# kaylode/vehicle-counting

Hardware: AMD Instinct MI355X
Metric: end-to-end frames/sec (detect+NMS+ReID+track), YOLOv5s 640px (higher is better)
Workload: dtype bf16; 1 GPU; YOLOv5s 640x640 single camera stream per GPU, bf16 convs (BASELINE.json configs[1]); workload_id=s640-bf16, clip_frames=512, objects=12, num_classes=80, detection_injection=False, weights=seeded synthetic (no checkpoints available), streams=1, ranks=1, counts_allgather_via=vc_allgather_counts (RCCL, C ABI), tracked_rows=155352, tracker=device-resident (one kernel per batch, no host round trip per frame)

## Files before the change

include/vcount_hip.h:

```cpp
#ifndef VCOUNT_HIP_H
#define VCOUNT_HIP_H

#include <stddef.h>
#include <stdint.h>

#ifdef __cplusplus
extern "C" {
#endif

#define VC_OK 0
#define VC_ERR_ARG 1
#define VC_ERR_HIP 2
#define VC_ERR_STATE 3
#define VC_ERR_CAPACITY 4
#define VC_ERR_NOTFOUND 5

#define VC_PREC_BF16 0
#define VC_PREC_F32 1
#define VC_PREC_FP8 2

#define VC_FEAT_DIM 512
#define VC_REID_SIZE 50

int vc_version(void);
// ... 88 lines not shown
    int full_range;
    int pitch_y, pitch_c;
    size_t offset_c, offset_v, frame_stride;
} vc_yuv_desc;
int vc_yuv_desc_default(vc_yuv_desc* d);
int vc_stream_stage_yuv_host(vc_engine* e, const vc_yuv_desc* d, const uint8_t* yuv_host, int b, int h, int w, void** frames_dev_out);
int vc_stream_stage_yuv_dev(vc_engine* e, const vc_yuv_desc* d, const void* yuv_dev, int b, int h, int w, void** frames_dev_out);
int vc_yuv_to_bgr_dev(const vc_yuv_desc* d, const void* yuv_dev, int b, int h, int w, void* bgr_dev);

int vc_stream_run_async(vc_engine* e, const int* trackers, int num_classes, const void* frames_dev, int b, int h, int w,
                        int cap_rows_per_frame);
int vc_stream_collect(vc_engine* e, int64_t* out_rows6, int cap_rows_per_frame, int* out_m, int* out_ndet, int b);
int vc_stream_run_async_multi(vc_engine* e, const int* trackers , int n_cam, int num_classes, const int* cam_of_frame ,
                              const void* frames_dev, int b, int h, int w, int cap_rows_per_frame);
int vc_stream_reset(vc_engine* e);

int vc_stream_embed(vc_engine* e, const void* frames_dev, int b, int h, int w, double* out_rows7, int cap_rows, int* out_n, const float** out_feat_dev);
int vc_allgather_rows(vc_engine* e, const double* rows7, const float* feat_dev, int n, double* out_rows7, int cap_rows, int* out_counts ,
                      const float** out_feat_dev);
int vc_videotracker_run_features(vc_engine* e, const int* trackers, int num_classes, const double* rows7, const float* feat_dev, int n, int h, int w,
                                 int64_t* out_rows6, int cap_rows_per_frame, int* out_m, int64_t* out_keys, int cap_frames, int* out_n_frames);
int vc_stream_inject(vc_engine* e, const float* det6 , const int* count, int b, int n);

typedef struct vc_counter vc_counter;
int vc_counter_create(const double* polygon_xy, int n_points, const double* dir_lines, int n_dir, int num_classes, vc_counter** out);
int vc_counter_destroy(vc_counter* c);
int vc_counter_add(vc_counter* c, const int64_t* frames, const int64_t* track_ids, const int64_t* labels, const int64_t* boxes_xyxy, int n);
int vc_counter_tracks(const vc_counter* c, int* n);
int vc_counts(const vc_counter* c, int32_t* out );
int vc_counter_rows_count(const vc_counter* c, int64_t* n);
// ... 74 lines not shown
```

vehicle-counting_amd/_lib.py:

```python
from __future__ import annotations

import ctypes as C
import os

import numpy as np

_HERE = os.path.dirname(os.path.abspath(__file__))
os.environ.setdefault("GPU_MAX_HW_QUEUES", "8")
LIB_PATH = os.environ.get("VC_LIB_PATH") or os.path.join(_HERE, "libvcount_hip.so")

VC_OK = 0
PREC_BF16, PREC_F32, PREC_FP8 = 0, 1, 2
PREC_ID = {"bf16": 0, "f32": 1, "fp8": 2}
NET_YOLO, NET_REID = 0, 1
FEAT_DIM = 512
PROF_CONV, PROF_DETECT_AUX, PROF_REID_AUX, PROF_TRACK = 0, 1, 2, 3
PIX_ID = {"nv12": 0, "i420": 1}
YUV_MATRIX_ID = {"bt601": 0, "bt709": 1}
RENDER_SRC_ID = {"bgr_host": 0, "bgr_dev": 1, "yuv_host": 2, "yuv_dev": 3}


class VcError(RuntimeError):
    def __init__(self, code, msg):
        super().__init__(f"libvcount_hip status {code}: {msg}")
# ... 72 lines not shown
    "vc_yuv_desc_default": [_P(YuvDesc)],
    "vc_stream_stage_yuv_host": [_vp, _P(YuvDesc), _vp, _i, _i, _i, _P(_vp)],
    "vc_stream_stage_yuv_dev": [_vp, _P(YuvDesc), _vp, _i, _i, _i, _P(_vp)],
    "vc_yuv_to_bgr_host": [_P(YuvDesc), _pu8, _i, _i, _i, _pu8],
    "vc_yuv_to_bgr_dev": [_P(YuvDesc), _vp, _i, _i, _i, _vp],
    "vc_bgr_to_yuv_host": [_P(YuvDesc), _pu8, _i, _i, _i, _pu8],
    "vc_bgr_to_yuv_dev": [_P(YuvDesc), _vp, _i, _i, _i, _vp],
    "vc_render_create": [_vp, _i, _i, _i, _i, _P(_vp)],
    "vc_render_destroy": [_vp],
    "vc_render_submit": [_vp, _P(RenderSrc), _i, _i, _i, _pi, _pi, _P(YuvDesc), _vp, _i],
    "vc_render_collect": [_vp],
    "vc_stream_run_async": [_vp, _pi, _i, _vp, _i, _i, _i, _i],
    "vc_stream_collect": [_vp, _pl, _i, _pi, _pi, _i],
    "vc_stream_run_async_multi": [_vp, _pi, _i, _i, _pi, _vp, _i, _i, _i, _i],
    "vc_stream_reset": [_vp],
    "vc_stream_embed": [_vp, _vp, _i, _i, _i, _pd, _i, _pi, _P(_vp)],
    "vc_allgather_rows": [_vp, _pd, _vp, _i, _pd, _i, _pi, _P(_vp)],
    "vc_videotracker_run_features": [_vp, _pi, _i, _pd, _vp, _i, _i, _i, _pl, _i, _pi, _pl, _i, _pi],
    "vc_counter_create": [_pd, _i, _pd, _i, _i, _P(_vp)],
    "vc_counter_destroy": [_vp],
    "vc_counter_add": [_vp, _pl, _pl, _pl, _pl, _i],
    "vc_counter_tracks": [_vp, _pi],
    "vc_counts": [_vp, _pi],
    "vc_counter_rows_count": [_vp, _pl],
    "vc_counter_rows": [_vp, C.c_int64, _pl, _pl, _pl, _pl, _pi, _pd, _pd, _pl, _pl],
    "vc_comm_unique_id": [_vp],
    "vc_comm_init": [_vp, _i, _i, _vp],
    "vc_comm_destroy": [_vp],
    "vc_allgather_counts": [_vp, _pi, _i, _pi],
    "vc_overlay": [_vp, _vp, _i, _i, _i, _pi, _pi],
# ... 68 lines not shown
```

vehicle-counting_amd/csrc/engine.h:

```cpp
#pragma once
#include <chrono>
#include <condition_variable>
#include <deque>
#include <map>
#include <mutex>
#include <memory>
#include <string>
#include <vector>

#include "kernels.h"

namespace vc {

struct ConvParam {
    std::string name;
    int O = 0, I = 0, kh = 0, kw = 0;
    bool set = false;
    bool pair_stem = false;
    int fuse_a = -1, fuse_b = -1;
    int obj_of = -1;
    bool hidden = false;
    std::vector<float> w, b;
    void* d_w = nullptr;
    float* d_scale = nullptr;
// ... 64 lines not shown
    std::vector<TrackTaskHost> tasks;
    std::vector<int> dev_index;
    std::vector<std::pair<int, int>> tracker_dets;
    std::vector<int> last_task_of;
};

struct YuvGeom {
    int nv12, h, w, pitch_y, pitch_c;
    size_t off_c, off_v, frame_stride, frame_end;
    int yoff, cy, cvr, cvg, cug, cub;
    int matrix, full_range;
};

}

struct vc_render;

struct vc_engine {
    vc_engine_config cfg{};
    int prec = 0;
    int aux_prec = 0;
    float act_scale = 1.0f;
    hipStream_t stream = nullptr;
    hipStream_t dstream = nullptr;
    hipStream_t rstream = nullptr;
    hipStream_t hstream = nullptr;
    hipEvent_t ev_fork = nullptr, ev_join = nullptr;
    void* d_zero = nullptr; size_t zero_bytes = 0; bool want_hc_count = false;
    hipEvent_t ev_det[2] = {nullptr, nullptr};
    hipEvent_t ev_reid[3] = {nullptr, nullptr, nullptr};
    bool finalized = false;
    struct Options { int c3_fused = 1, bneck_fused = 1, bneck_cv3 = 1, front_fused = 1, crop_per_pixel = 0, sparse_head = 1, ff_ablate = 0, c3_ablate = 0, reid_block_fused = 1, head_side = 1, fuse_upsample = 1, sppf_sep = 1, fuse_s2_pw = 1; } opt;
    std::vector<void*> allocs;
    std::vector<void*> host_allocs;

    vc::Net yolo;
    int ch[5] = {0, 0, 0, 0, 0}, rep[4] = {0, 0, 0, 0};
    std::map<std::string, vc::View> ybuf;
    const vc::YoloPlan* last_plan = nullptr;
    std::vector<vc::ConvP> s2pw_folded;
    std::vector<std::pair<vc::View, vc::View>> up_folded;
    std::map<std::vector<int>, vc::YoloPlan> yolo_plans;
    std::map<std::pair<int, int>, vc::ReidPlan> reid_plans;
    uint8_t* d_frames = nullptr;
    size_t d_frames_bytes = 0;
    float* d_logits[3] = {nullptr, nullptr, nullptr};
    void* d_obj[3] = {nullptr, nullptr, nullptr};
// ... 22 lines not shown
    float* h_geom = nullptr;
    unsigned geom_seq = 0, submit_seq = 0;
    hipStream_t cstream = nullptr;
    uint8_t* d_ingest[4] = {nullptr, nullptr, nullptr, nullptr};
    hipEvent_t ev_ingest[4] = {nullptr, nullptr, nullptr, nullptr};
    unsigned ingest_seq = 0;
    bool ingest_staged[4] = {false, false, false, false};
    uint8_t* d_yuv_raw[4] = {nullptr, nullptr, nullptr, nullptr};
    size_t yuv_raw_bytes[4] = {0, 0, 0, 0};
    float* d_feat2[3] = {nullptr, nullptr, nullptr};
    int* d_crops2[3] = {nullptr, nullptr, nullptr};
    int* h_crops2[3] = {nullptr, nullptr, nullptr};
    unsigned reid_seq = 0;
    std::vector<int> crop_scratch;
    struct FrameDets { std::vector<double> xyxy, conf; std::vector<int> label; };
    struct Pending {
        const void* frames; int b, h, w, slot;
        int stage = 0;
        bool embed_refused = false;
        int fslot = 0;
        std::vector<FrameDets> fd;
        std::vector<int> row0;
        std::vector<float> inj_det; std::vector<int> inj_cnt; int inj_b = 0, inj_n = 0;
    };
    std::vector<Pending> pending;
    struct AsyncJob { int stage = 0, b = 0, cap = 0; std::vector<int> ndet; const void* frames = nullptr; };
    std::deque<AsyncJob> jobs;

    vc::Net reid;
    std::map<std::string, vc::View> rbuf;
    int* d_crops = nullptr;
    int* h_crops = nullptr;
    float* d_feat = nullptr;
    float* h_feat = nullptr;
    float* d_reid_in_nchw = nullptr;

    vc::TrackPool pool{};
// ... 76 lines not shown
int ingest_publish(vc_engine* e, int slot, void** frames_dev_out);
int yuv_resolve(const vc_yuv_desc* d, int b, int h, int w, YuvGeom& g);
size_t yuv_batch_bytes(const YuvGeom& g, int b);
int launch_yuv_to_bgr(const YuvGeom& g, const uint8_t* src, uint8_t* dst, int b, hipStream_t s);
int launch_bgr_to_yuv(const YuvGeom& g, const uint8_t* src_bgr, uint8_t* dst_yuv, int b, hipStream_t s);
int overlay_check_lists(int b, const int32_t* prims12, const int32_t* frame_first);
int launch_overlay(uint8_t* frames_dev, int b, int h, int w, const void* d_prims, const int* d_first, hipStream_t s);
void render_destroy_all(vc_engine* e);
struct ProfScope {
    vc_engine* e; int cat; double flops, bytes;
    hipStream_t s;
    ProfScope(vc_engine* e_, int cat_, double flops_ = 0, double bytes_ = 0, hipStream_t s_ = nullptr);
    ~ProfScope();
};
int tracker_init_pool(vc_engine* e);
struct Prepared { std::vector<double> tlwh, conf; std::vector<int> feat_rows; };
void prepare_dets(const double* xyxy, const double* conf, const int* rows, int k, const vc_tracker_params& p, Prepared& out);
void dsort_nms(const double* tlwh, const double* scores, int n, double max_overlap, std::vector<int>& keep);
struct FrameClassDets { int label, tracker; Prepared dets; };
int track_enqueue(vc_engine* e, int st, const std::vector<std::vector<FrameClassDets>>& frames, const float* d_feat, int W, int H,
                  int rows_cap, hipEvent_t wait);
int track_collect(vc_engine* e, int st, int64_t* out_rows6, int cap_rows_per_frame, int* out_m);
int track_idle(vc_engine* e);
int async_wait_all(vc_engine* e);
int frame_track(vc_engine* e, const uint8_t* d_frame_base, int frame_index, int H, int W, const std::vector<int>& tracker_ids,
                const std::vector<int>& labels, const std::vector<std::vector<int>>& groups, const double* xyxy, const double* conf,
                int n, std::vector<int64_t>& rows6);
}
```

vehicle-counting_amd/csrc/engine.hip:

```cpp
#include <algorithm>
#include <cmath>
#include <cstdarg>
#include <cstdlib>

#include "engine.h"

namespace vc {

static thread_local char g_err[1024] = "";
void set_error(const char* fmt, ...) {
    va_list ap;
    va_start(ap, fmt);
    vsnprintf(g_err, sizeof(g_err), fmt, ap);
    va_end(ap);
}
const char* last_error() { return g_err; }

int dev_alloc(vc_engine* e, void** p, size_t bytes) {
    if (bytes == 0) bytes = 16;
    VC_HIP(hipMalloc(p, bytes));
    e->allocs.push_back(*p);
    return VC_OK;
}
int dev_realloc(vc_engine* e, void** p, size_t bytes) {
// ... 128 lines not shown
    }
    int ndev = 0;
    VC_HIP(hipGetDeviceCount(&ndev));
    VC_CHECK(cfg->device >= 0 && cfg->device < ndev, VC_ERR_HIP, "device %d not present (%d visible)", cfg->device, ndev);
    VC_HIP(hipSetDevice(cfg->device));
    vc_engine* e = new vc_engine();
    e->cfg = *cfg;
    e->prec = cfg->precision;
    e->aux_prec = cfg->precision == VC_PREC_FP8 ? (int)PREC_BF16 : cfg->precision;
    e->act_scale = getenv("VC_FP8_ACT_SCALE") ? (float)atof(getenv("VC_FP8_ACT_SCALE")) : 1.0f;
    {
        auto env_int = [](const char* name, int dflt) { const char* v = getenv(name); return v ? atoi(v) : dflt; };
        e->opt.c3_fused = env_int("VC_C3_FUSED", 1); e->opt.bneck_fused = env_int("VC_BNECK_FUSED", 1); e->opt.bneck_cv3 = env_int("VC_BNECK_CV3", 1);
        e->opt.front_fused = env_int("VC_FRONT_FUSED", 1); e->opt.crop_per_pixel = getenv("VC_CROP_PER_PIXEL") ? 1 : 0;
        e->opt.sparse_head = env_int("VC_SPARSE_HEAD", 1); e->opt.reid_block_fused = env_int("VC_REID_BLOCK_FUSED", 1); e->opt.head_side = env_int("VC_HEAD_SIDE", 1); e->opt.fuse_upsample = env_int("VC_FUSE_UPSAMPLE", 1); e->opt.sppf_sep = env_int("VC_SPPF_SEP", 1); e->opt.fuse_s2_pw = env_int("VC_FUSE_S2PW", 1);
    }
    memcpy(e->anchors, kAnchors, sizeof(kAnchors));
    int st = VC_OK;
    do {
        int plo = 0, phi = 0;
        hipDeviceGetStreamPriorityRange(&plo, &phi);
        const int reserve = getenv("VC_TRACK_CUS") ? atoi(getenv("VC_TRACK_CUS")) : 0;
        bool ok;
        if (reserve > 0) {
            hipDeviceProp_t prop;
            hipGetDeviceProperties(&prop, cfg->device);
            const int ncu = prop.multiProcessorCount, words = (ncu + 31) / 32;
            std::vector<uint32_t> mt(words, 0), mc(words, 0);
            for (int c = 0; c < ncu; ++c) (c < reserve ? mt : mc)[c / 32] |= 1u << (c % 32);
            ok = hipExtStreamCreateWithCUMask(&e->stream, words, mt.data()) == hipSuccess &&
// ... 139 lines not shown
    }
    for (auto& p : e->reid.params) VC_TRY(pack_and_upload(e, p, e->aux_prec));
    e->d_frames_bytes = (size_t)e->cfg.max_batch * e->cfg.max_frame_h * e->cfg.max_frame_w * 3;
    VC_TRY(dev_alloc(e, (void**)&e->d_frames, e->d_frames_bytes));
    if (e->cfg.with_detector) VC_TRY(yolo_alloc(e));
    if (e->cfg.with_reid) VC_TRY(reid_alloc(e));
    for (auto& p : e->yolo.params) { p.w.clear(); p.w.shrink_to_fit(); }
    for (auto& p : e->reid.params) { p.w.clear(); p.w.shrink_to_fit(); }
    e->finalized = true;
    return VC_OK;
}

int vc_engine_set_option(vc_engine* e, const char* name, int value) {
    VC_CHECK(e && name, VC_ERR_ARG, "null argument");
    const std::string n = name;
    if (n == "c3_fused") e->opt.c3_fused = value;
    else if (n == "bneck_fused") e->opt.bneck_fused = value;
    else if (n == "bneck_cv3") e->opt.bneck_cv3 = value;
    else if (n == "front_fused") e->opt.front_fused = value;
    else if (n == "crop_per_pixel") e->opt.crop_per_pixel = value;
    else if (n == "sparse_head") e->opt.sparse_head = value;
    else if (n == "reid_block_fused") e->opt.reid_block_fused = value;
    else if (n == "head_side") e->opt.head_side = value;
    else if (n == "fuse_upsample") e->opt.fuse_upsample = value;
    else if (n == "sppf_sep") e->opt.sppf_sep = value;
    else if (n == "fuse_s2_pw") e->opt.fuse_s2_pw = value;
    else if (n == "ff_ablate") e->opt.ff_ablate = value;
    else if (n == "c3_ablate") e->opt.c3_ablate = value;
    else if (n == "dot_arena_mb") { VC_CHECK(value >= 0, VC_ERR_ARG, "dot_arena_mb must be >= 0"); e->dot_arena_max_floats = (size_t)value * 262144; }
    else { set_error("unknown option '%s'", name); return VC_ERR_NOTFOUND; }
// ... 407 lines not shown
```

vehicle-counting_amd/csrc/stream.hip:

```cpp
#include <algorithm>
#include <cmath>
#include <numeric>

#include <chrono>
#include <cstdlib>
#include <thread>

#include "engine.h"

using namespace vc;

namespace {
struct Tm {
    double acc[8] = {0, 0, 0, 0, 0, 0, 0, 0};
    long calls = 0;
    std::chrono::steady_clock::time_point t;
    bool on = getenv("VC_TIMING") != nullptr;
    void start() { if (on) t = std::chrono::steady_clock::now(); }
    void lap(int i) {
        if (!on) return;
        auto n = std::chrono::steady_clock::now();
        acc[i] += std::chrono::duration<double, std::micro>(n - t).count();
        t = n;
    }
// ... 103 lines not shown
    VC_TRY(ingest_take_slot(e, b, h, w, &slot));
    VC_HIP(hipMemcpyAsync(e->d_ingest[slot], frames_host, (size_t)b * h * w * 3, hipMemcpyHostToDevice, e->cstream));
    return ingest_publish(e, slot, frames_dev_out);
}

int vc_stream_submit_host(vc_engine* e, const uint8_t* frames_host, int b, int h, int w, void** frames_dev_out) {
    VC_CHECK(e && e->pending.size() < 2, e ? VC_ERR_STATE : VC_ERR_ARG, "two submissions are already in flight: call vc_stream_run first");
    VC_TRY(vc_stream_stage_host(e, frames_host, b, h, w, frames_dev_out));
    return vc_stream_submit(e, *frames_dev_out, b, h, w);
}

}

namespace {

int issue_reid(vc_engine* e, vc_engine::Pending& pd) {
    const int md = e->cfg.max_det, b = pd.b, h = pd.h, w = pd.w;
    const float* h_det = e->h_det2[pd.slot];
    const int* h_cnt = e->h_det_count2[pd.slot];
    pd.fd.assign(b, FrameDets{});
    pd.row0.assign(b, 0);
    for (int f = 0; f < b; ++f) {
        VC_CHECK(h_cnt[f] >= 0 || pd.inj_b > 0, VC_ERR_CAPACITY, "frame %d: more than max_candidates (%d) boxes passed conf_thres; raise vc_engine_config.max_candidates", f,
                 e->cfg.max_candidates);
        if (pd.inj_b > 0) {
            const int fi = f % pd.inj_b;
            marshal(pd.inj_det.data() + (size_t)fi * pd.inj_n * 6, pd.inj_cnt[fi], pd.fd[f]);
        } else {
            marshal(h_det + (size_t)f * md * 6, h_cnt[f], pd.fd[f]);
        }
    }
    std::vector<int>& crops = e->crop_scratch;
    crops.clear();
    int k = 0;
    for (int f = 0; f < b; ++f) {
        pd.row0[f] = k;
        FrameDets& d = pd.fd[f];
        VC_CHECK(k + (int)d.conf.size() <= e->cfg.max_crops, VC_ERR_CAPACITY,
                 "the batch has more boxes than max_crops (%d): raise vc_engine_config.max_crops", e->cfg.max_crops);
        for (size_t i = 0; i < d.conf.size(); ++i) {
            const double* bx = &d.xyxy[i * 4];
            const double bw = bx[2] - bx[0], bh = bx[3] - bx[1];
            const double cx = bx[0] + bw / 2, cy = bx[1] + bh / 2;
            int c[5];
            c[0] = f;
            c[1] = std::max((int)(cx - bw / 2), 0); c[3] = std::min((int)(cx + bw / 2), w - 1);
            c[2] = std::max((int)(cy - bh / 2), 0); c[4] = std::min((int)(cy + bh / 2), h - 1);
            VC_CHECK(c[3] > c[1] && c[4] > c[2], VC_ERR_ARG,
                     "frame %d box %zu gives an empty crop (the reference's cv2.resize raises here)", f, i);
            crops.insert(crops.end(), c, c + 5);
            ++k;
        }
    }
    pd.fslot = (int)(e->reid_seq++ % 3);
    int* hc = e->h_crops2[pd.fslot];
    if (k > 0) {
        memcpy(hc, crops.data(), (size_t)k * 5 * sizeof(int));
        VC_HIP(hipMemcpyAsync(e->d_crops2[pd.fslot], hc, (size_t)k * 5 * sizeof(int), hipMemcpyHostToDevice, e->rstream));
        VC_TRY(run_reid_on(e, (const uint8_t*)pd.frames, h, w, k, e->d_crops2[pd.fslot], e->d_feat2[pd.fslot], e->rstream));
    }
    VC_HIP(hipEventRecord(e->ev_reid[pd.fslot], e->rstream));
    pd.stage = 1;
    return VC_OK;
}

int issue_reid_or_drop(vc_engine* e, size_t idx) {
    const int st = issue_reid(e, e->pending[idx]);
    if (st != VC_OK) e->pending.erase(e->pending.begin() + idx);
    return st;
}

void try_issue_next(vc_engine* e) {
    int next = -1;
    int embedded = 0;
    for (size_t i = 0; i < e->pending.size(); ++i) {
        if (e->pending[i].stage == 0) { next = (int)i; break; }
        ++embedded;
    }
    if (next < 0 || e->pending[next].embed_refused) return;
    embedded += (int)e->jobs.size();
    if (embedded >= 3) return;
    if (hipEventQuery(e->ev_det[e->pending[next].slot]) != hipSuccess) return;
    if (issue_reid(e, e->pending[next]) != VC_OK) e->pending[next].embed_refused = true;
}

}

extern "C" {

static int enqueue_batch_tracking(vc_engine* e, vc_engine::Pending& pd, const int* all_trackers, int num_classes, const int* cam_of_frame, int n_cam,
                                  int stage, int cap_rows_per_frame, std::vector<int>& ndet) {
    const int b = pd.b;
    ndet.assign(b, 0);
    std::vector<std::vector<FrameClassDets>> frames(b);
    std::vector<std::vector<int>> by_class(num_classes);
    for (int f = 0; f < b; ++f) {
        const int cam = cam_of_frame ? cam_of_frame[f] : 0;
        VC_CHECK(cam >= 0 && cam < n_cam, VC_ERR_ARG, "frame %d: camera index %d outside [0, %d)", f, cam, n_cam);
        const int* trackers = all_trackers + (size_t)cam * num_classes;
        FrameDets& d = pd.fd[f];
        ndet[f] = (int)d.conf.size();
        if (d.conf.empty()) continue;
        for (size_t i = 0; i < d.label.size(); ++i)
            if (d.label[i] >= 0 && d.label[i] < num_classes) by_class[d.label[i]].push_back((int)i);
        for (int c = 0; c < num_classes; ++c) {
            std::vector<int>& g = by_class[c];
            if (g.empty()) continue;
            const int ts = tracker_slot(e->trackers, trackers[c]);
            VC_CHECK(ts >= 0, VC_ERR_NOTFOUND, "bad or stale tracker handle %d for class %d", trackers[c], c);
            std::vector<double> bx(g.size() * 4), cf(g.size());
            std::vector<int> rows(g.size());
            for (size_t i = 0; i < g.size(); ++i) {
                memcpy(&bx[i * 4], &d.xyxy[(size_t)g[i] * 4], 4 * sizeof(double));
                cf[i] = d.conf[g[i]];
                rows[i] = pd.row0[f] + g[i];
            }
            FrameClassDets fc{c, ts, {}};
// ... 33 lines not shown
}

extern "C" {

int vc_stream_run_async(vc_engine* e, const int* trackers, int num_classes, const void* frames_dev, int b, int h, int w,
                        int cap_rows_per_frame) {
    return vc_stream_run_async_multi(e, trackers, 1, num_classes, nullptr, frames_dev, b, h, w, cap_rows_per_frame);
}

int vc_stream_run_async_multi(vc_engine* e, const int* trackers, int n_cam, int num_classes, const int* cam_of_frame, const void* frames_dev, int b, int h,
                              int w, int cap_rows_per_frame) {
    VC_CHECK(e && trackers && frames_dev && cap_rows_per_frame > 0 && n_cam >= 1 && (n_cam == 1 || cam_of_frame), VC_ERR_ARG, "bad argument");
    VC_CHECK(e->finalized && e->cfg.with_detector && e->cfg.with_reid, VC_ERR_STATE, "engine not finalized");
    VC_HIP(hipSetDevice(e->cfg.device));
    VC_CHECK(e->jobs.size() < 2, VC_ERR_STATE, "two asynchronous batches are already outstanding: call vc_stream_collect");
    vc_engine::Pending pd;
    VC_TRY(take_front(e, frames_dev, b, h, w, pd));
    vc_engine::AsyncJob job;
    job.stage = (int)(e->tstage_seq++ % 3); job.b = b; job.cap = cap_rows_per_frame; job.frames = frames_dev;
    VC_TRY(enqueue_batch_tracking(e, pd, trackers, num_classes, cam_of_frame, n_cam, job.stage, cap_rows_per_frame, job.ndet));
    e->jobs.push_back(std::move(job));
    g_tm.report();
    try_issue_next(e);
    return VC_OK;
}

int vc_stream_collect(vc_engine* e, int64_t* out_rows6, int cap_rows_per_frame, int* out_m, int* out_ndet, int b) {
    VC_CHECK(e && out_rows6 && out_m, VC_ERR_ARG, "null argument");
    VC_HIP(hipSetDevice(e->cfg.device));
    VC_CHECK(!e->jobs.empty(), VC_ERR_STATE, "no asynchronous batch is outstanding");
// ... 11 lines not shown
    return VC_OK;
}

int vc_stream_run(vc_engine* e, const int* trackers, int num_classes, const void* frames_dev, int b, int h, int w,
                  int64_t* out_rows6, int cap_rows_per_frame, int* out_m, int* out_ndet) {
    VC_CHECK(e && trackers && frames_dev && out_rows6 && out_m, VC_ERR_ARG, "null argument");
    VC_CHECK(e->jobs.empty(), VC_ERR_STATE, "asynchronous batches are outstanding: vc_stream_collect them first");
    VC_TRY(vc_stream_run_async(e, trackers, num_classes, frames_dev, b, h, w, cap_rows_per_frame));
    return vc_stream_collect(e, out_rows6, cap_rows_per_frame, out_m, out_ndet, b);
}

int vc_stream_embed(vc_engine* e, const void* frames_dev, int b, int h, int w, double* out_rows7, int cap_rows, int* out_n, const float** out_feat_dev) {
    VC_CHECK(e && frames_dev && out_rows7 && out_n && out_feat_dev, VC_ERR_ARG, "null argument");
    VC_CHECK(e->finalized && e->cfg.with_detector && e->cfg.with_reid, VC_ERR_STATE, "engine not finalized");
    VC_HIP(hipSetDevice(e->cfg.device));
    vc_engine::Pending pd;
    VC_TRY(take_front(e, frames_dev, b, h, w, pd));
    VC_HIP(hipEventSynchronize(e->ev_reid[pd.fslot]));
    int n = 0;
    for (int f = 0; f < b; ++f) n += (int)pd.fd[f].conf.size();
    VC_CHECK(n <= cap_rows, VC_ERR_CAPACITY, "vc_stream_embed: %d rows, room for %d", n, cap_rows);
    double* o = out_rows7;
    for (int f = 0; f < b; ++f) {
        const FrameDets& d = pd.fd[f];
        for (size_t i = 0; i < d.conf.size(); ++i, o += 7) {
            o[0] = (double)f; memcpy(o + 1, &d.xyxy[i * 4], 4 * sizeof(double)); o[5] = d.conf[i]; o[6] = (double)d.label[i];
        }
    }
    *out_n = n;
    *out_feat_dev = e->d_feat2[pd.fslot];
    return VC_OK;
}
// ... 45 lines not shown

int vc_stream_reset(vc_engine* e) {
    VC_CHECK(e, VC_ERR_ARG, "null engine");
    VC_HIP(hipSetDevice(e->cfg.device));
    VC_HIP(hipStreamSynchronize(e->dstream)); VC_HIP(hipStreamSynchronize(e->rstream)); VC_HIP(hipStreamSynchronize(e->stream));
    while (!e->jobs.empty()) {
        const vc_engine::AsyncJob job = std::move(e->jobs.front());
        e->jobs.pop_front();
        std::vector<int64_t> rows((size_t)job.b * job.cap * 6);
        std::vector<int> m(job.b);
        (void)track_collect(e, job.stage, rows.data(), job.cap, m.data());
    }
    e->pending.clear();
    if (e->cstream) VC_HIP(hipStreamSynchronize(e->cstream));
    for (bool& st : e->ingest_staged) st = false;
    return VC_OK;
}

namespace {
struct P2 { double x, y; };
inline int orient(P2 p, P2 q, P2 r) {
    const double v = (q.y - p.y) * (r.x - q.x) - (q.x - p.x) * (r.y - q.y);
    return v == 0 ? 0 : (v > 0 ? 1 : 2);
}
inline bool on_segment(P2 p, P2 q, P2 r) {
    return q.x <= std::max(p.x, r.x) && q.x >= std::min(p.x, r.x) && q.y <= std::max(p.y, r.y) && q.y >= std::min(p.y, r.y);
}
inline bool intersect(P2 p1, P2 q1, P2 p2, P2 q2) {
    const int o1 = orient(p1, q1, p2), o2 = orient(p1, q1, q2), o3 = orient(p2, q2, p1), o4 = orient(p2, q2, q1);
    if (o1 != o2 && o3 != o4) return true;
// ... 70 lines not shown
```

vehicle-counting_amd/csrc/tracker.hip:

```cpp
#include <algorithm>
#include <cstring>
#include <cmath>
#include <numeric>
#include <climits>
#include <cstdint>
#include <cstdlib>

#include "engine.h"
#include "track_core.h"

namespace vc {

using namespace tc;

void dsort_nms(const double* tlwh, const double* scores, int n, double max_overlap, std::vector<int>& keep) {
    keep.clear();
    if (n == 0) return;
    std::vector<double> x1(n), y1(n), x2(n), y2(n), area(n);
    for (int i = 0; i < n; ++i) {
        x1[i] = tlwh[i * 4]; y1[i] = tlwh[i * 4 + 1]; x2[i] = tlwh[i * 4 + 2] + tlwh[i * 4]; y2[i] = tlwh[i * 4 + 3] + tlwh[i * 4 + 1];
        area[i] = (x2[i] - x1[i] + 1) * (y2[i] - y1[i] + 1);
    }
    std::vector<int> idx(n);
    std::iota(idx.begin(), idx.end(), 0);
// ... 1 lines not shown
    while (!idx.empty()) {
        const int i = idx.back();
        idx.pop_back();
        keep.push_back(i);
        std::vector<int> rest;
        for (int j : idx) {
            const double w = std::max(0.0, std::min(x2[i], x2[j]) - std::max(x1[i], x1[j]) + 1);
            const double h = std::max(0.0, std::min(y2[i], y2[j]) - std::max(y1[i], y1[j]) + 1);
            if (!((w * h) / area[j] > max_overlap)) rest.push_back(j);
        }
        idx.swap(rest);
    }
}

void prepare_dets(const double* xyxy, const double* conf, const int* rows, int k, const vc_tracker_params& p, Prepared& out) {
    std::vector<double> tl, cf;
    std::vector<int> fr;
    for (int i = 0; i < k; ++i) {
        if (!(conf[i] > p.min_confidence)) continue;
        const double* b = xyxy + (size_t)i * 4;
        const double w = b[2] - b[0], h = b[3] - b[1];
        const double cx = b[0] + w / 2, cy = b[1] + h / 2;
        tl.push_back(cx - w / 2.); tl.push_back(cy - h / 2.); tl.push_back(w); tl.push_back(h);
        cf.push_back(conf[i]);
        fr.push_back(rows[i]);
    }
    std::vector<int> keep;
    dsort_nms(tl.data(), cf.data(), (int)cf.size(), p.nms_max_overlap, keep);
    out.tlwh.clear(); out.conf.clear(); out.feat_rows.clear();
    for (int i : keep) {
        for (int c = 0; c < 4; ++c) out.tlwh.push_back(tl[(size_t)i * 4 + c]);
        out.conf.push_back(cf[i]);
        out.feat_rows.push_back(fr[i]);
    }
}

static size_t align16(size_t x) { return (x + 15) & ~(size_t)15; }

int tracker_init_pool(vc_engine* e) {
    const size_t T = e->cfg.max_tracks, S = e->cfg.nn_budget_cap;
    VC_CHECK(T >= 1 && S >= 1, VC_ERR_ARG, "max_tracks and nn_budget_cap must be positive");
    e->max_trackers = e->cfg.max_trackers > 0 ? e->cfg.max_trackers : 256;
    VC_CHECK(e->max_trackers <= 65535, VC_ERR_ARG, "max_trackers %d: a tracker handle addresses at most 65535 slots", e->max_trackers);
// ... 298 lines not shown

static void xyxy_to_cxcywh(const double* b, double* o) {
    const double w = b[2] - b[0], h = b[3] - b[1];
    o[0] = b[0] + w / 2; o[1] = b[1] + h / 2; o[2] = w; o[3] = h;
}

static void crop_corners_i(const double* b, int W, int H, int* c) {
    c[0] = std::max((int)(b[0] - b[2] / 2), 0); c[2] = std::min((int)(b[0] + b[2] / 2), W - 1);
    c[1] = std::max((int)(b[1] - b[3] / 2), 0); c[3] = std::min((int)(b[1] + b[3] / 2), H - 1);
}

int frame_track(vc_engine* e, const uint8_t* d_frame_base, int frame_index, int H, int W, const std::vector<int>& tracker_ids,
                const std::vector<int>& labels, const std::vector<std::vector<int>>& groups, const double* xyxy, const double* conf,
                int n, std::vector<int64_t>& rows6) {
    VC_CHECK(n <= e->cfg.max_crops, VC_ERR_CAPACITY, "%d crops exceed max_crops %d", n, e->cfg.max_crops);
    for (int i = 0; i < n; ++i) {
        double c[4]; int q[4];
        xyxy_to_cxcywh(xyxy + (size_t)i * 4, c);
        crop_corners_i(c, W, H, q);
        VC_CHECK(q[2] > q[0] && q[3] > q[1], VC_ERR_ARG, "box %d gives an empty crop (the reference's cv2.resize raises here)", i);
        int* h = e->h_crops + (size_t)i * 5;
        h[0] = frame_index; h[1] = q[0]; h[2] = q[1]; h[3] = q[2]; h[4] = q[3];
    }
    VC_HIP(hipMemcpyAsync(e->d_crops, e->h_crops, (size_t)n * 5 * sizeof(int), hipMemcpyHostToDevice, e->stream));
    VC_TRY(run_reid_dev(e, d_frame_base, H, W, n));
    std::vector<std::vector<FrameClassDets>> frames(1);
    int total_tracks = 0;
    for (size_t j = 0; j < tracker_ids.size(); ++j) {
        const auto& g = groups[j];
        std::vector<double> bx(g.size() * 4), cf(g.size());
        std::vector<int> rows(g.size());
        for (size_t i = 0; i < g.size(); ++i) {
            memcpy(&bx[i * 4], xyxy + (size_t)g[i] * 4, 4 * sizeof(double));
            cf[i] = conf[g[i]];
            rows[i] = g[i];
        }
        const int ts = tracker_slot(e->trackers, tracker_ids[j]);
        VC_CHECK(ts >= 0, VC_ERR_NOTFOUND, "bad or stale tracker handle %d", tracker_ids[j]);
        FrameClassDets fc{labels[j], ts, {}};
        prepare_dets(bx.data(), cf.data(), rows.data(), (int)g.size(), e->trackers[ts]->p, fc.dets);
        total_tracks += e->trackers[ts]->known_tracks + (int)fc.dets.conf.size();
        frames[0].push_back(std::move(fc));
    }
    const int cap = std::max(total_tracks, 16);
    VC_TRY(track_enqueue(e, 3, frames, e->d_feat, W, H, cap, nullptr));
    std::vector<int64_t> buf((size_t)cap * 6);
    int m = 0;
    VC_TRY(track_collect(e, 3, buf.data(), cap, &m));
    rows6.assign(buf.begin(), buf.begin() + (size_t)m * 6);
    return VC_OK;
}

struct HostTrackerState { TrackerHdr hdr; std::vector<int> list; std::vector<TrackRecD> recs; };

static int download_tracker(vc_engine* e, int id, HostTrackerState& st) {
    VC_TRY(track_idle(e));
    VC_HIP(hipStreamSynchronize(e->stream));
// ... 471 lines not shown
```

vehicle-counting_amd/engine.py:

```python
from __future__ import annotations

import ctypes as C

import numpy as np

from . import _lib as L
from .weights import fold_reid

YOLO_VARIANT_ID = {"yolov5s": 0, "yolov5m": 1, "yolov5l": 2}


class Engine:

    def __init__(self, yolo_sd=None, reid_sd=None, *, device=0, precision="bf16", model_name="yolov5s", num_classes=80,
                 img_size=640, max_batch=16, max_frame_hw=(720, 1280), conf_thres=0.25, iou_thres=0.45, max_det=300,
                 max_candidates=4096, max_crops=1024, max_tracks=4096, nn_budget_cap=100, max_trackers=256):
        lib = L.lib()
        cfg = L.EngineConfig()
        L.check(lib.vc_engine_config_default(C.byref(cfg)))
        cfg.device = device
        cfg.precision = L.PREC_ID[precision]
        cfg.yolo_variant = YOLO_VARIANT_ID[model_name]
        cfg.num_classes, cfg.img_size, cfg.max_batch = num_classes, img_size, max_batch
        cfg.max_frame_h, cfg.max_frame_w = max_frame_hw
# ... 42 lines not shown
        try:
            self.close()
        except Exception:
            pass

    def sync(self):
        L.check(L.lib().vc_engine_sync(self._h))

    def set_option(self, name, value):
        L.check(L.lib().vc_engine_set_option(self._h, name.encode(), int(value)))

    def stream_reset(self):
        L.check(L.lib().vc_stream_reset(self._h))
        self._async_shapes = []

    def detect(self, imgs_rgb):
        n = len(imgs_rgb)
        imgs = [np.ascontiguousarray(im, dtype=np.uint8) for im in imgs_rgb]
        ptrs = (C.c_void_p * n)(*[im.ctypes.data for im in imgs])
        hs = (C.c_int * n)(*[im.shape[0] for im in imgs])
        ws = (C.c_int * n)(*[im.shape[1] for im in imgs])
        md = self.cfg.max_det
        out = np.zeros((n, md, 6), np.float32)
        cnt = np.zeros(n, np.int32)
        L.check(L.lib().vc_detect(self._h, ptrs, hs, ws, n, L.ptr(out, C.c_float), L.ptr(cnt, C.c_int)))
        return [out[i, :cnt[i]].copy() for i in range(n)]

    def debug_layer(self, layer, batch=1):
        dims = (C.c_int * 4)()
        cap = batch * max(640, int(self.cfg.img_size)) ** 2 * 32
# ... 471 lines not shown
```

Baseline: 21610 frames/s.

## Embed only detections that survive tracker confidence and NMS filtering

Before issuing ReID, the stream path now runs the tracker's min_confidence filter and DeepSORT NMS per frame and class on the host, and compacts the crop list to the surviving boxes. The embedding network then runs on fewer crops, and feature row indices are remapped. If the tracker parameters at track time differ from the ones used for filtering, it falls back to re-embedding all crops. The trade is extra host-side grouping and NMS work moved earlier, plus a possible re-embed path, in exchange for less ReID GPU work.

```diff
diff --git a/include/vcount_hip.h b/include/vcount_hip.h
--- a/include/vcount_hip.h
+++ b/include/vcount_hip.h
@@ -126,6 +126,7 @@
 int vc_stream_run_async_multi(vc_engine* e, const int* trackers , int n_cam, int num_classes, const int* cam_of_frame ,
                               const void* frames_dev, int b, int h, int w, int cap_rows_per_frame);
 int vc_stream_reset(vc_engine* e);
+int vc_stream_crop_stats(vc_engine* e, int64_t* boxes_detected, int64_t* crops_embedded);
 
 int vc_stream_embed(vc_engine* e, const void* frames_dev, int b, int h, int w, double* out_rows7, int cap_rows, int* out_n, const float** out_feat_dev);
 int vc_allgather_rows(vc_engine* e, const double* rows7, const float* feat_dev, int n, double* out_rows7, int cap_rows, int* out_counts ,
diff --git a/vehicle-counting_amd/_lib.py b/vehicle-counting_amd/_lib.py
--- a/vehicle-counting_amd/_lib.py
+++ b/vehicle-counting_amd/_lib.py
@@ -110,6 +110,7 @@
     "vc_stream_collect": [_vp, _pl, _i, _pi, _pi, _i],
     "vc_stream_run_async_multi": [_vp, _pi, _i, _i, _pi, _vp, _i, _i, _i, _i],
     "vc_stream_reset": [_vp],
+    "vc_stream_crop_stats": [_vp, _P(C.c_int64), _P(C.c_int64)],
     "vc_stream_embed": [_vp, _vp, _i, _i, _i, _pd, _i, _pi, _P(_vp)],
     "vc_allgather_rows": [_vp, _pd, _vp, _i, _pd, _i, _pi, _P(_vp)],
     "vc_videotracker_run_features": [_vp, _pi, _i, _pd, _vp, _i, _i, _i, _pl, _i, _pi, _pl, _i, _pi],
diff --git a/vehicle-counting_amd/csrc/engine.h b/vehicle-counting_amd/csrc/engine.h
--- a/vehicle-counting_amd/csrc/engine.h
+++ b/vehicle-counting_amd/csrc/engine.h
@@ -102,6 +102,10 @@
 
 }
 
+namespace vc {
+struct Prepared { std::vector<double> tlwh, conf; std::vector<int> feat_rows; };
+}
+
 struct vc_render;
 
 struct vc_engine {
@@ -118,7 +122,7 @@
     hipEvent_t ev_det[2] = {nullptr, nullptr};
     hipEvent_t ev_reid[3] = {nullptr, nullptr, nullptr};
     bool finalized = false;
-    struct Options { int c3_fused = 1, bneck_fused = 1, bneck_cv3 = 1, front_fused = 1, crop_per_pixel = 0, sparse_head = 1, ff_ablate = 0, c3_ablate = 0, reid_block_fused = 1, head_side = 1, fuse_upsample = 1, sppf_sep = 1, fuse_s2_pw = 1; } opt;
+    struct Options { int c3_fused = 1, bneck_fused = 1, bneck_cv3 = 1, front_fused = 1, crop_per_pixel = 0, sparse_head = 1, ff_ablate = 0, c3_ablate = 0, reid_block_fused = 1, head_side = 1, fuse_upsample = 1, sppf_sep = 1, fuse_s2_pw = 1, embed_kept_only = 1; } opt;
     std::vector<void*> allocs;
     std::vector<void*> host_allocs;
 
@@ -171,6 +175,9 @@
     unsigned reid_seq = 0;
     std::vector<int> crop_scratch;
     struct FrameDets { std::vector<double> xyxy, conf; std::vector<int> label; };
+    struct EmbedFilter { bool valid = false; double min_confidence = 0, nms_max_overlap = 0; };
+    EmbedFilter stream_flt;
+    long long boxes_detected = 0, crops_embedded = 0;
     struct Pending {
         const void* frames; int b, h, w, slot;
         int stage = 0;
@@ -178,6 +185,9 @@
         int fslot = 0;
         std::vector<FrameDets> fd;
         std::vector<int> row0;
+        bool filtered = false;
+        EmbedFilter flt;
+        std::vector<std::vector<std::pair<int, vc::Prepared>>> prep;
         std::vector<float> inj_det; std::vector<int> inj_cnt; int inj_b = 0, inj_n = 0;
     };
     std::vector<Pending> pending;
@@ -284,8 +294,8 @@
     ~ProfScope();
 };
 int tracker_init_pool(vc_engine* e);
-struct Prepared { std::vector<double> tlwh, conf; std::vector<int> feat_rows; };
 void prepare_dets(const double* xyxy, const double* conf, const int* rows, int k, const vc_tracker_params& p, Prepared& out);
+void prepare_dets(const double* xyxy, const double* conf, const int* rows, int k, double min_confidence, double nms_max_overlap, Prepared& out);
 void dsort_nms(const double* tlwh, const double* scores, int n, double max_overlap, std::vector<int>& keep);
 struct FrameClassDets { int label, tracker; Prepared dets; };
 int track_enqueue(vc_engine* e, int st, const std::vector<std::vector<FrameClassDets>>& frames, const float* d_feat, int W, int H,
diff --git a/vehicle-counting_amd/csrc/engine.hip b/vehicle-counting_amd/csrc/engine.hip
--- a/vehicle-counting_amd/csrc/engine.hip
+++ b/vehicle-counting_amd/csrc/engine.hip
@@ -166,6 +166,7 @@
         e->opt.c3_fused = env_int("VC_C3_FUSED", 1); e->opt.bneck_fused = env_int("VC_BNECK_FUSED", 1); e->opt.bneck_cv3 = env_int("VC_BNECK_CV3", 1);
         e->opt.front_fused = env_int("VC_FRONT_FUSED", 1); e->opt.crop_per_pixel = getenv("VC_CROP_PER_PIXEL") ? 1 : 0;
         e->opt.sparse_head = env_int("VC_SPARSE_HEAD", 1); e->opt.reid_block_fused = env_int("VC_REID_BLOCK_FUSED", 1); e->opt.head_side = env_int("VC_HEAD_SIDE", 1); e->opt.fuse_upsample = env_int("VC_FUSE_UPSAMPLE", 1); e->opt.sppf_sep = env_int("VC_SPPF_SEP", 1); e->opt.fuse_s2_pw = env_int("VC_FUSE_S2PW", 1);
+        e->opt.embed_kept_only = env_int("VC_EMBED_KEPT_ONLY", 1);
     }
     memcpy(e->anchors, kAnchors, sizeof(kAnchors));
     int st = VC_OK;
@@ -335,6 +336,7 @@
 int vc_engine_set_option(vc_engine* e, const char* name, int value) {
     VC_CHECK(e && name, VC_ERR_ARG, "null argument");
     const std::string n = name;
+    if (n == "embed_kept_only") { e->opt.embed_kept_only = value; return VC_OK; }
     if (n == "c3_fused") e->opt.c3_fused = value;
     else if (n == "bneck_fused") e->opt.bneck_fused = value;
     else if (n == "bneck_cv3") e->opt.bneck_cv3 = value;
diff --git a/vehicle-counting_amd/csrc/stream.hip b/vehicle-counting_amd/csrc/stream.hip
--- a/vehicle-counting_amd/csrc/stream.hip
+++ b/vehicle-counting_amd/csrc/stream.hip
@@ -1,5 +1,6 @@
 #include <algorithm>
 #include <cmath>
+#include <map>
 #include <numeric>
 
 #include <chrono>
@@ -141,24 +142,10 @@
 
 namespace {
 
-int issue_reid(vc_engine* e, vc_engine::Pending& pd) {
-    const int md = e->cfg.max_det, b = pd.b, h = pd.h, w = pd.w;
-    const float* h_det = e->h_det2[pd.slot];
-    const int* h_cnt = e->h_det_count2[pd.slot];
-    pd.fd.assign(b, FrameDets{});
+int all_crops(vc_engine* e, vc_engine::Pending& pd, std::vector<int>& crops) {
+    const int b = pd.b, h = pd.h, w = pd.w;
+    crops.clear();
     pd.row0.assign(b, 0);
-    for (int f = 0; f < b; ++f) {
-        VC_CHECK(h_cnt[f] >= 0 || pd.inj_b > 0, VC_ERR_CAPACITY, "frame %d: more than max_candidates (%d) boxes passed conf_thres; raise vc_engine_config.max_candidates", f,
-                 e->cfg.max_candidates);
-        if (pd.inj_b > 0) {
-            const int fi = f % pd.inj_b;
-            marshal(pd.inj_det.data() + (size_t)fi * pd.inj_n * 6, pd.inj_cnt[fi], pd.fd[f]);
-        } else {
-            marshal(h_det + (size_t)f * md * 6, h_cnt[f], pd.fd[f]);
-        }
-    }
-    std::vector<int>& crops = e->crop_scratch;
-    crops.clear();
     int k = 0;
     for (int f = 0; f < b; ++f) {
         pd.row0[f] = k;
@@ -179,20 +166,94 @@
             ++k;
         }
     }
-    pd.fslot = (int)(e->reid_seq++ % 3);
+    return VC_OK;
+}
+
+int enqueue_reid(vc_engine* e, vc_engine::Pending& pd, const int* crops, int k) {
     int* hc = e->h_crops2[pd.fslot];
     if (k > 0) {
-        memcpy(hc, crops.data(), (size_t)k * 5 * sizeof(int));
+        memcpy(hc, crops, (size_t)k * 5 * sizeof(int));
         VC_HIP(hipMemcpyAsync(e->d_crops2[pd.fslot], hc, (size_t)k * 5 * sizeof(int), hipMemcpyHostToDevice, e->rstream));
-        VC_TRY(run_reid_on(e, (const uint8_t*)pd.frames, h, w, k, e->d_crops2[pd.fslot], e->d_feat2[pd.fslot], e->rstream));
+        VC_TRY(run_reid_on(e, (const uint8_t*)pd.frames, pd.h, pd.w, k, e->d_crops2[pd.fslot], e->d_feat2[pd.fslot], e->rstream));
     }
     VC_HIP(hipEventRecord(e->ev_reid[pd.fslot], e->rstream));
+    e->crops_embedded += k;
+    return VC_OK;
+}
+
+int issue_reid(vc_engine* e, vc_engine::Pending& pd, const vc_engine::EmbedFilter& flt) {
+    const int md = e->cfg.max_det, b = pd.b;
+    const float* h_det = e->h_det2[pd.slot];
+    const int* h_cnt = e->h_det_count2[pd.slot];
+    pd.fd.assign(b, FrameDets{});
+    for (int f = 0; f < b; ++f) {
+        VC_CHECK(h_cnt[f] >= 0 || pd.inj_b > 0, VC_ERR_CAPACITY, "frame %d: more than max_candidates (%d) boxes passed conf_thres; raise vc_engine_config.max_candidates", f,
+                 e->cfg.max_candidates);
+        if (pd.inj_b > 0) {
+            const int fi = f % pd.inj_b;
+            marshal(pd.inj_det.data() + (size_t)fi * pd.inj_n * 6, pd.inj_cnt[fi], pd.fd[f]);
+        } else {
+            marshal(h_det + (size_t)f * md * 6, h_cnt[f], pd.fd[f]);
+        }
+    }
+    std::vector<int>& crops = e->crop_scratch;
+    VC_TRY(all_crops(e, pd, crops));
+    int k = (int)(crops.size() / 5);
+    e->boxes_detected += k;
+    pd.filtered = e->opt.embed_kept_only != 0 && flt.valid;
+    pd.flt = flt;
+    pd.prep.clear();
+    if (pd.filtered) {
+        pd.prep.resize(b);
+        std::map<int, std::vector<int>> by_label;
+        std::vector<int> row_of;
+        std::vector<double> bx, cf;
+        int kept = 0;
+        for (int f = 0; f < b; ++f) {
+            const FrameDets& d = pd.fd[f];
+            const int nf = (int)d.conf.size();
+            by_label.clear();
+            for (int i = 0; i < nf; ++i) by_label[d.label[i]].push_back(i);
+            row_of.assign(nf, -1);
+            for (auto& lg : by_label) {
+                const std::vector<int>& g = lg.second;
+                bx.resize(g.size() * 4); cf.resize(g.size());
+                for (size_t i = 0; i < g.size(); ++i) {
+                    memcpy(&bx[i * 4], &d.xyxy[(size_t)g[i] * 4], 4 * sizeof(double));
+                    cf[i] = d.conf[g[i]];
+                }
+                pd.prep[f].emplace_back(lg.first, Prepared{});
+                Prepared& pr = pd.prep[f].back().second;
+                prepare_dets(bx.data(), cf.data(), g.data(), (int)g.size(), flt.min_confidence, flt.nms_max_overlap, pr);
+                for (int r : pr.feat_rows) row_of[r] = 0;
+            }
+            for (int i = 0; i < nf; ++i)
+                if (row_of[i] == 0) {
+                    memmove(&crops[(size_t)kept * 5], &crops[(size_t)(pd.row0[f] + i) * 5], 5 * sizeof(int));
+                    row_of[i] = kept++;
+                }
+            for (auto& lp : pd.prep[f])
+                for (int& r : lp.second.feat_rows) r = row_of[r];
+        }
+        k = kept;
+    }
+    pd.fslot = (int)(e->reid_seq++ % 3);
+    VC_TRY(enqueue_reid(e, pd, crops.data(), k));
     pd.stage = 1;
     return VC_OK;
 }
 
+int reembed_unfiltered(vc_engine* e, vc_engine::Pending& pd) {
+    VC_HIP(hipEventSynchronize(e->ev_reid[pd.fslot]));
+    std::vector<int>& crops = e->crop_scratch;
+    VC_TRY(all_crops(e, pd, crops));
+    pd.filtered = false;
+    pd.prep.clear();
+    return enqueue_reid(e, pd, crops.data(), (int)(crops.size() / 5));
+}
+
 int issue_reid_or_drop(vc_engine* e, size_t idx) {
-    const int st = issue_reid(e, e->pending[idx]);
+    const int st = issue_reid(e, e->pending[idx], e->stream_flt);
     if (st != VC_OK) e->pending.erase(e->pending.begin() + idx);
     return st;
 }
@@ -208,7 +269,7 @@
     embedded += (int)e->jobs.size();
     if (embedded >= 3) return;
     if (hipEventQuery(e->ev_det[e->pending[next].slot]) != hipSuccess) return;
-    if (issue_reid(e, e->pending[next]) != VC_OK) e->pending[next].embed_refused = true;
+    if (issue_reid(e, e->pending[next], e->stream_flt) != VC_OK) e->pending[next].embed_refused = true;
 }
 
 }
@@ -219,15 +280,42 @@
                                   int stage, int cap_rows_per_frame, std::vector<int>& ndet) {
     const int b = pd.b;
     ndet.assign(b, 0);
+    for (int f = 0; f < b; ++f) {
+        const int cam = cam_of_frame ? cam_of_frame[f] : 0;
+        VC_CHECK(cam >= 0 && cam < n_cam, VC_ERR_ARG, "frame %d: camera index %d outside [0, %d)", f, cam, n_cam);
+    }
+    if (pd.filtered) {
+        bool same = true;
+        for (int f = 0; f < b && same; ++f) {
+            const int* trackers = all_trackers + (size_t)(cam_of_frame ? cam_of_frame[f] : 0) * num_classes;
+            for (const auto& lp : pd.prep[f]) {
+                if (lp.first < 0 || lp.first >= num_classes) continue;
+                const int ts = tracker_slot(e->trackers, trackers[lp.first]);
+                if (ts < 0) continue;
+                const vc_tracker_params& p = e->trackers[ts]->p;
+                if (p.min_confidence != pd.flt.min_confidence || p.nms_max_overlap != pd.flt.nms_max_overlap) { same = false; break; }
+            }
+        }
+        if (!same) VC_TRY(reembed_unfiltered(e, pd));
+    }
     std::vector<std::vector<FrameClassDets>> frames(b);
     std::vector<std::vector<int>> by_class(num_classes);
     for (int f = 0; f < b; ++f) {
         const int cam = cam_of_frame ? cam_of_frame[f] : 0;
-        VC_CHECK(cam >= 0 && cam < n_cam, VC_ERR_ARG, "frame %d: camera index %d outside [0, %d)", f, cam, n_cam);
         const int* trackers = all_trackers + (size_t)cam * num_classes;
         FrameDets& d = pd.fd[f];
         ndet[f] = (int)d.conf.size();
         if (d.conf.empty()) continue;
+        if (pd.filtered) {
+            for (auto& lp : pd.prep[f]) {
+                const int c = lp.first;
+                if (c < 0 || c >= num_classes) continue;
+                const int ts = tracker_slot(e->trackers, trackers[c]);
+                VC_CHECK(ts >= 0, VC_ERR_NOTFOUND, "bad or stale tracker handle %d for class %d", trackers[c], c);
+                frames[f].push_back(FrameClassDets{c, ts, std::move(lp.second)});
+            }
+            continue;
+        }
         for (size_t i = 0; i < d.label.size(); ++i)
             if (d.label[i] >= 0 && d.label[i] < num_classes) by_class[d.label[i]].push_back((int)i);
         for (int c = 0; c < num_classes; ++c) {
@@ -291,6 +379,17 @@
     VC_CHECK(e->finalized && e->cfg.with_detector && e->cfg.with_reid, VC_ERR_STATE, "engine not finalized");
     VC_HIP(hipSetDevice(e->cfg.device));
     VC_CHECK(e->jobs.size() < 2, VC_ERR_STATE, "two asynchronous batches are already outstanding: call vc_stream_collect");
+    {
+        vc_engine::EmbedFilter flt;
+        for (int i = 0; i < n_cam * num_classes; ++i) {
+            const int ts = tracker_slot(e->trackers, trackers[i]);
+            if (ts < 0) { flt.valid = false; break; }
+            const vc_tracker_params& p = e->trackers[ts]->p;
+            if (i == 0) { flt.valid = true; flt.min_confidence = p.min_confidence; flt.nms_max_overlap = p.nms_max_overlap; }
+            else if (p.min_confidence != flt.min_confidence || p.nms_max_overlap != flt.nms_max_overlap) { flt.valid = false; break; }
+        }
+        e->stream_flt = flt;
+    }
     vc_engine::Pending pd;
     VC_TRY(take_front(e, frames_dev, b, h, w, pd));
     vc_engine::AsyncJob job;
@@ -332,8 +431,10 @@
     VC_CHECK(e && frames_dev && out_rows7 && out_n && out_feat_dev, VC_ERR_ARG, "null argument");
     VC_CHECK(e->finalized && e->cfg.with_detector && e->cfg.with_reid, VC_ERR_STATE, "engine not finalized");
     VC_HIP(hipSetDevice(e->cfg.device));
+    e->stream_flt = vc_engine::EmbedFilter{};
     vc_engine::Pending pd;
     VC_TRY(take_front(e, frames_dev, b, h, w, pd));
+    if (pd.filtered) VC_TRY(reembed_unfiltered(e, pd));
     VC_HIP(hipEventSynchronize(e->ev_reid[pd.fslot]));
     int n = 0;
     for (int f = 0; f < b; ++f) n += (int)pd.fd[f].conf.size();
@@ -409,6 +510,15 @@
     e->pending.clear();
     if (e->cstream) VC_HIP(hipStreamSynchronize(e->cstream));
     for (bool& st : e->ingest_staged) st = false;
+    e->stream_flt = vc_engine::EmbedFilter{};
+    e->boxes_detected = e->crops_embedded = 0;
+    return VC_OK;
+}
+
+int vc_stream_crop_stats(vc_engine* e, int64_t* boxes_detected, int64_t* crops_embedded) {
+    VC_CHECK(e && boxes_detected && crops_embedded, VC_ERR_ARG, "null argument");
+    *boxes_detected = e->boxes_detected;
+    *crops_embedded = e->crops_embedded;
     return VC_OK;
 }
 
diff --git a/vehicle-counting_amd/csrc/tracker.hip b/vehicle-counting_amd/csrc/tracker.hip
--- a/vehicle-counting_amd/csrc/tracker.hip
+++ b/vehicle-counting_amd/csrc/tracker.hip
@@ -39,10 +39,14 @@
 }
 
 void prepare_dets(const double* xyxy, const double* conf, const int* rows, int k, const vc_tracker_params& p, Prepared& out) {
+    prepare_dets(xyxy, conf, rows, k, p.min_confidence, p.nms_max_overlap, out);
+}
+
+void prepare_dets(const double* xyxy, const double* conf, const int* rows, int k, double min_confidence, double nms_max_overlap, Prepared& out) {
     std::vector<double> tl, cf;
     std::vector<int> fr;
     for (int i = 0; i < k; ++i) {
-        if (!(conf[i] > p.min_confidence)) continue;
+        if (!(conf[i] > min_confidence)) continue;
         const double* b = xyxy + (size_t)i * 4;
         const double w = b[2] - b[0], h = b[3] - b[1];
         const double cx = b[0] + w / 2, cy = b[1] + h / 2;
@@ -51,7 +55,7 @@
         fr.push_back(rows[i]);
     }
     std::vector<int> keep;
-    dsort_nms(tl.data(), cf.data(), (int)cf.size(), p.nms_max_overlap, keep);
+    dsort_nms(tl.data(), cf.data(), (int)cf.size(), nms_max_overlap, keep);
     out.tlwh.clear(); out.conf.clear(); out.feat_rows.clear();
     for (int i : keep) {
         for (int c = 0; c < 4; ++c) out.tlwh.push_back(tl[(size_t)i * 4 + c]);
@@ -380,16 +384,15 @@
                 const std::vector<int>& labels, const std::vector<std::vector<int>>& groups, const double* xyxy, const double* conf,
                 int n, std::vector<int64_t>& rows6) {
     VC_CHECK(n <= e->cfg.max_crops, VC_ERR_CAPACITY, "%d crops exceed max_crops %d", n, e->cfg.max_crops);
+    std::vector<int> crops((size_t)n * 5);
     for (int i = 0; i < n; ++i) {
         double c[4]; int q[4];
         xyxy_to_cxcywh(xyxy + (size_t)i * 4, c);
         crop_corners_i(c, W, H, q);
         VC_CHECK(q[2] > q[0] && q[3] > q[1], VC_ERR_ARG, "box %d gives an empty crop (the reference's cv2.resize raises here)", i);
-        int* h = e->h_crops + (size_t)i * 5;
+        int* h = &crops[(size_t)i * 5];
         h[0] = frame_index; h[1] = q[0]; h[2] = q[1]; h[3] = q[2]; h[4] = q[3];
     }
-    VC_HIP(hipMemcpyAsync(e->d_crops, e->h_crops, (size_t)n * 5 * sizeof(int), hipMemcpyHostToDevice, e->stream));
-    VC_TRY(run_reid_dev(e, d_frame_base, H, W, n));
     std::vector<std::vector<FrameClassDets>> frames(1);
     int total_tracks = 0;
     for (size_t j = 0; j < tracker_ids.size(); ++j) {
@@ -407,6 +410,23 @@
         prepare_dets(bx.data(), cf.data(), rows.data(), (int)g.size(), e->trackers[ts]->p, fc.dets);
         total_tracks += e->trackers[ts]->known_tracks + (int)fc.dets.conf.size();
         frames[0].push_back(std::move(fc));
+    }
+    int k = n;
+    if (e->opt.embed_kept_only) {
+        std::vector<int> row_of(n, -1);
+        for (const FrameClassDets& fc : frames[0])
+            for (int r : fc.dets.feat_rows) row_of[r] = 0;
+        k = 0;
+        for (int i = 0; i < n; ++i)
+            if (row_of[i] == 0) { memmove(&crops[(size_t)k * 5], &crops[(size_t)i * 5], 5 * sizeof(int)); row_of[i] = k++; }
+        for (FrameClassDets& fc : frames[0])
+            for (int& r : fc.dets.feat_rows) r = row_of[r];
+    }
+    e->boxes_detected += n; e->crops_embedded += k;
+    if (k > 0) {
+        memcpy(e->h_crops, crops.data(), (size_t)k * 5 * sizeof(int));
+        VC_HIP(hipMemcpyAsync(e->d_crops, e->h_crops, (size_t)k * 5 * sizeof(int), hipMemcpyHostToDevice, e->stream));
+        VC_TRY(run_reid_dev(e, d_frame_base, H, W, k));
     }
     const int cap = std::max(total_tracks, 16);
     VC_TRY(track_enqueue(e, 3, frames, e->d_feat, W, H, cap, nullptr));
diff --git a/vehicle-counting_amd/engine.py b/vehicle-counting_amd/engine.py
--- a/vehicle-counting_amd/engine.py
+++ b/vehicle-counting_amd/engine.py
@@ -80,6 +80,11 @@
         L.check(L.lib().vc_stream_reset(self._h))
         self._async_shapes = []
 
+    def stream_crop_stats(self):
+        boxes, crops = C.c_int64(), C.c_int64()
+        L.check(L.lib().vc_stream_crop_stats(self._h, C.byref(boxes), C.byref(crops)))
+        return boxes.value, crops.value
+
     def detect(self, imgs_rgb):
         n = len(imgs_rgb)
         imgs = [np.ascontiguousarray(im, dtype=np.uint8) for im in imgs_rgb]
```

Result: faster. 22380 frames/s (median of 6 runs) (+3.5%).
